# ClashLuke/LocAtE

Hardware: AMD Instinct MI355X
Metric: images/sec (G+D step) 64x64 bs=64 (higher is better)
Workload: dtype f32 (contractions fp32-faithful on the matrix cores: 2 x scaled fp16 operand pieces / 3 MFMAs per slice where the operand's largest magnitude comes with it, else 3 x bf16 pieces / 6 MFMAs; fp32 accumulate); 1 GPU; LocAtE G+D step, 64x64 RGB, batch 64 per GPU (the fp32 variant - the reference's own precision - of BASELINE.json configs[1]: 64x64 RGB bs 64), self/feature attention at 16x16 and 64x64, random-init weights; global_batch=64, image_size=64, parallelism=dp1, launch=hipGraph replay, G-step generator pass on a second stream

## Files before the change

include/locate_hip.h:

```cpp
#ifndef LOCATE_HIP_H
#define LOCATE_HIP_H
#include <stddef.h>
#include <stdint.h>
#ifdef __cplusplus
extern "C" {
#endif

const char* locate_last_error(void);
int locate_abi_version(void);
int locate_device_info(char* arch_name, int name_len, int* cu_count, int* wave_size);

int locate_roottanh_fwd(const float* x, float* y, int64_t n, void* absmax , void* stream);
int locate_absmax_words(void);
int locate_roottanh_bwd(const float* x, const float* gy, float* gx, int64_t n, int accumulate, void* absmax, void* stream);
int locate_absmax(const float* x, int64_t n, void* absmax, void* stream);
int locate_act_cat_rows_fwd(const float* latent, const float* pre, float* out, int rows, int z, int w, void* stream);
int locate_act_rows_bwd(const float* pre, const float* g, int64_t g_row_stride, const float* g_add, float* gpre, int rows, int w,
                        void* stream);
int locate_add3(const float* a, int64_t a_bs, const float* b, int64_t b_bs, const float* c, int64_t c_bs, float* out, int batch,
                int64_t per, void* stream);
int locate_tanh_fwd(const float* x, float* y, int64_t n, void* stream);
int locate_tanh_bwd(const float* y, const float* gy, float* gx, int64_t n, void* stream);

size_t locate_norm_stats_workspace_bytes(void);
// ... 47 lines not shown
                         const float* wv, float* gw, float* du, float* dsigma_out, int h, int wd, void* stream);
size_t locate_sn_group_workspace_bytes(void);
int locate_sn_weight_bwd_grouped(const float* gy, int64_t gy_bs, const float* y, int64_t y_bs, const float* bias, int groups,
                                 int Bg, int M, int plane, const float* sigma_tab, int sigma_stride, const float* u,
                                 const float* v, const float* wv, int64_t wv_stride, float* gw, float* du,
                                 float* dsigma_total_out, int h, int wd, void* workspace, void* stream);
int locate_sn_dv_batched(const void* table, int n_layers, int max_h, int max_wd, void* stream);

size_t locate_conv_panel_bytes(const int* geom, int adjoint);
int locate_conv_pack_panel(const int* geom, int adjoint, const float* w, float* panel, void* stream);
size_t locate_conv_pack_job_bytes(void);
int locate_conv_pack_job(const int* geom, int adjoint, const float* w, float* panel, int block_start, void* job_out,
                         int* blocks_out, int direct, const void* weight_absmax);
int locate_conv_pack_panels(const void* jobs, int n_jobs, int total_blocks, int any_f16, int passes, void* stream);
int locate_conv_pack_job_is_direct(const void* job);
int locate_conv_pack_job_is_window(const void* job);
int locate_conv_win_ok(const int* geom, int adjoint_fmt, int64_t x_bs, const void* x);
size_t locate_conv_win_workspace_bytes(const int* geom, int adjoint_fmt);
size_t locate_conv_fwd_workspace_bytes(const int* geom);
size_t locate_conv_counter_bytes(void);
int locate_conv_fwd(const int* geom, const float* x, int64_t x_bs, const float* panel, const float* scale,
                    int scale_group_batch, int scale_stride, const float* bias, float* y, int64_t y_bs, void* workspace,
                    void* counters, int precision, const void* x_absmax, const void* act_epilogue, void* stream);
size_t locate_conv_dgrad_workspace_bytes(const int* geom);
int locate_conv_dgrad(const int* geom, const float* gy, int64_t gy_bs, const float* panel, const float* scale,
                      int scale_group_batch, int scale_stride, const float* bias, float* gx, int64_t gx_bs, void* workspace,
                      void* counters, int precision, const void* gy_absmax, const void* act_epilogue, void* stream);
size_t locate_conv_wgrad_workspace_bytes(const int* geom);
int locate_conv_wgrad_partials(const int* geom);
int locate_conv_wgrad(const int* geom, const float* x, int64_t x_bs, const float* gy, int64_t gy_bs, float* gw,
                      const float* w_ref, const float* inv_scale, int scale_group_batch, int scale_stride,
                      double* inner_partial, void* workspace, int precision, const void* x_absmax, const void* gy_absmax,
                      void* deferred_reduce, void* stream);
int locate_conv_wgrad_group_partials(const int* geom, int groups);
size_t locate_conv_wgrad_group_workspace_bytes(const int* geom, int groups);
size_t locate_slab_reduce_record_bytes(void);
int locate_slab_reduce_max(void);
int locate_slab_reduce_record_blocks(const void* record);
int locate_slab_reduce_batch(const void* records, int n, void* stream);

size_t locate_wgrad_batch_record_bytes(void);
int locate_wgrad_batch_max(void);
int locate_wgrad_batch_record(const int* geom, const float* x, int64_t x_bs, const float* gy, int64_t gy_bs, float* gw,
                              const float* w_ref, const float* inv_scale, int scale_group_batch, int scale_stride,
                              double* inner_partial, void* record);
int locate_wgrad_batch(const void* records, int n, void* stream);

int locate_dwconv_fwd(const int* geom, const float* x, int64_t x_bs, const float* w, const float* scale, int scale_group_batch,
                      int scale_stride, float* y, int64_t y_bs, void* stream);
int locate_dwconv_dgrad(const int* geom, const float* gy, int64_t gy_bs, const float* w, const float* scale,
                        int scale_group_batch, int scale_stride, float* gx, int64_t gx_bs, void* stream);
size_t locate_dwconv_wgrad_workspace_bytes(const int* geom);
int locate_dwconv_wgrad_partials(const int* geom);
int locate_dwconv_wgrad(const int* geom, const float* big, int64_t big_bs, const float* small, int64_t small_bs, float* gw,
                        const float* w_ref, const float* inv_scale, int scale_group_batch, int scale_stride,
                        double* inner_partial, void* workspace, void* stream);
int locate_groupdot_fwd(const float* x, int64_t x_bs, const float* w, const float* scale, int scale_group_batch,
                        int scale_stride, float* y, int B, int G, int L, void* stream);
int locate_groupdot_dgrad(const float* gy, const float* w, const float* scale, int scale_group_batch, int scale_stride,
                          float* gx, int64_t gx_bs, int B, int G, int L, void* stream);
int locate_groupdot_wgrad_partials(int G, int L);
int locate_groupdot_wgrad(const float* x, int64_t x_bs, const float* gy, float* gw, const float* w_ref, const float* inv_scale,
                          int scale_group_batch, int scale_stride, double* inner_partial, int B, int G, int L, void* stream);

size_t locate_fin_record_bytes(void);
int locate_fin_sn_dot_partials(int Bg, int M, int plane);
// ... 49 lines not shown
```

locate_amd/_lib.py:

```python
import ctypes
import os

import torch

_HERE = os.path.dirname(os.path.abspath(__file__))
LIB_PATH = os.path.join(_HERE, "csrc", "liblocate_hip_dbg.so" if os.environ.get("LOCATE_HIP_DEBUG_LIBRARY") == "1"
                        else "liblocate_hip.so")

c_p = ctypes.c_void_p
c_i = ctypes.c_int
c_i64 = ctypes.c_int64
c_f = ctypes.c_float
c_d = ctypes.c_double
c_sz = ctypes.c_size_t
c_ip = ctypes.POINTER(ctypes.c_int)

PROTOTYPES = {
    "locate_last_error": (ctypes.c_char_p, []),
    "locate_abi_version": (c_i, []),
    "locate_device_info": (c_i, [ctypes.c_char_p, c_i, c_ip, c_ip]),
    "locate_roottanh_fwd": (c_i, [c_p, c_p, c_i64, c_p, c_p]),
    "locate_roottanh_bwd": (c_i, [c_p, c_p, c_p, c_i64, c_i, c_p, c_p]),
    "locate_act_cat_rows_fwd": (c_i, [c_p, c_p, c_p, c_i, c_i, c_i, c_p]),
    "locate_act_rows_bwd": (c_i, [c_p, c_p, c_i64, c_p, c_p, c_i, c_i, c_p]),
# ... 28 lines not shown
    "locate_pool2_upsample2x_fwd": (c_i, [c_p, c_p, c_i64, c_i, c_i, c_p]),
    "locate_pool2_upsample2x_bwd": (c_i, [c_p, c_p, c_i64, c_i, c_i, c_i, c_p]),
    "locate_avgpool2_fwd": (c_i, [c_p, c_p, c_i64, c_i, c_i, c_p]),
    "locate_avgpool2_bwd": (c_i, [c_p, c_p, c_i64, c_i, c_i, c_i, c_p]),
    "locate_feature_pool_fwd": (c_i, [c_p, c_p, c_i64, c_i, c_p]),
    "locate_feature_pool_bwd": (c_i, [c_p, c_p, c_i64, c_i, c_i, c_p]),
    "locate_copy_channels": (c_i, [c_p, c_p, c_i, c_i, c_i, c_i64, c_i64, c_i, c_p]),
    "locate_sn_workspace_bytes": (c_sz, [c_i, c_i]),
    "locate_sn_power_iter": (c_i, [c_p, c_p, c_p, c_p, c_p, c_i, c_i, c_p, c_p]),
    "locate_sn_table_record_bytes": (c_sz, []),
    "locate_sn_power_iter_batched": (c_i, [c_p, c_i, c_i, c_i, c_p]),
    "locate_sn_weight_bwd": (c_i, [c_p, c_i, c_p, c_p, c_p, c_p, c_p, c_p, c_p, c_i, c_i, c_p]),
    "locate_sn_group_workspace_bytes": (c_sz, []),
    "locate_sn_weight_bwd_grouped": (c_i, [c_p, c_i64, c_p, c_i64, c_p, c_i, c_i, c_i, c_i, c_p, c_i, c_p, c_p, c_p, c_i64, c_p,
                                           c_p, c_p, c_i, c_i, c_p, c_p]),
    "locate_sn_dv_batched": (c_i, [c_p, c_i, c_i, c_i, c_p]),
    "locate_conv_panel_bytes": (c_sz, [c_ip, c_i]),
    "locate_conv_pack_panel": (c_i, [c_ip, c_i, c_p, c_p, c_p]),
    "locate_conv_pack_job_bytes": (c_sz, []),
    "locate_conv_pack_job": (c_i, [c_ip, c_i, c_p, c_p, c_i, c_p, c_ip, c_i, c_p]),
    "locate_conv_pack_panels": (c_i, [c_p, c_i, c_i, c_i, c_i, c_p]),
    "locate_conv_pack_job_is_direct": (c_i, [c_p]),
    "locate_conv_pack_job_is_window": (c_i, [c_p]),
    "locate_conv_win_ok": (c_i, [c_ip, c_i, c_i64, c_p]),
    "locate_conv_win_workspace_bytes": (c_sz, [c_ip, c_i]),
    "locate_conv_fwd_workspace_bytes": (c_sz, [c_ip]),
    "locate_conv_counter_bytes": (c_sz, []),
    "locate_conv_fwd": (c_i, [c_ip, c_p, c_i64, c_p, c_p, c_i, c_i, c_p, c_p, c_i64, c_p, c_p, c_i, c_p, c_p, c_p]),
    "locate_conv_dgrad_workspace_bytes": (c_sz, [c_ip]),
    "locate_conv_dgrad": (c_i, [c_ip, c_p, c_i64, c_p, c_p, c_i, c_i, c_p, c_p, c_i64, c_p, c_p, c_i, c_p, c_p, c_p]),
    "locate_conv_wgrad_workspace_bytes": (c_sz, [c_ip]),
    "locate_conv_wgrad_partials": (c_i, [c_ip]),
    "locate_conv_wgrad": (c_i, [c_ip, c_p, c_i64, c_p, c_i64, c_p, c_p, c_p, c_i, c_i, c_p, c_p, c_i, c_p, c_p, c_p, c_p]),
    "locate_conv_wgrad_group_partials": (c_i, [c_ip, c_i]),
    "locate_conv_wgrad_group_workspace_bytes": (c_sz, [c_ip, c_i]),
    "locate_slab_reduce_record_bytes": (c_sz, []),
    "locate_slab_reduce_max": (c_i, []),
    "locate_slab_reduce_record_blocks": (c_i, [c_p]),
    "locate_slab_reduce_batch": (c_i, [c_p, c_i, c_p]),
    "locate_dwconv_fwd": (c_i, [c_ip, c_p, c_i64, c_p, c_p, c_i, c_i, c_p, c_i64, c_p]),
    "locate_dwconv_dgrad": (c_i, [c_ip, c_p, c_i64, c_p, c_p, c_i, c_i, c_p, c_i64, c_p]),
    "locate_dwconv_wgrad_workspace_bytes": (c_sz, [c_ip]),
    "locate_dwconv_wgrad_partials": (c_i, [c_ip]),
    "locate_dwconv_wgrad": (c_i, [c_ip, c_p, c_i64, c_p, c_i64, c_p, c_p, c_p, c_i, c_i, c_p, c_p, c_p]),
    "locate_groupdot_fwd": (c_i, [c_p, c_i64, c_p, c_p, c_i, c_i, c_p, c_i, c_i, c_i, c_p]),
    "locate_groupdot_dgrad": (c_i, [c_p, c_p, c_p, c_i, c_i, c_p, c_i64, c_i, c_i, c_i, c_p]),
    "locate_groupdot_wgrad_partials": (c_i, [c_i, c_i]),
    "locate_groupdot_wgrad": (c_i, [c_p, c_i64, c_p, c_p, c_p, c_p, c_i, c_i, c_p, c_i, c_i, c_i, c_p]),
    "locate_fin_record_bytes": (c_sz, []),
    "locate_fin_sn_dot_partials": (c_i, [c_i, c_i, c_i]),
    "locate_fin_sn_dots": (c_i, [c_p, c_i, c_p]),
    "locate_fin_sn_rank1": (c_i, [c_p, c_i, c_p]),
    "locate_fin_sums": (c_i, [c_p, c_i, c_p]),
    "locate_fin_channel_slices": (c_i, [c_i, c_i, c_i]),
    "locate_fin_channel_sums": (c_i, [c_p, c_i, c_p]),
    "locate_gate_bwd_partials": (c_i, [c_i64, c_i]),
    "locate_multi_copy_record_bytes": (c_sz, []),
    "locate_multi_copy_chunk_elems": (c_i, []),
    "locate_multi_copy": (c_i, [c_p, c_p, c_i, c_i, c_f, c_p]),
    "locate_nadam_tensor_record_bytes": (c_sz, []),
    "locate_nadam_chunk_elems": (c_i, []),
    "locate_nadam_step": (c_i, [c_p, c_p, c_p, c_i, c_i, c_d, c_d, c_d, c_d, c_d, c_d, c_p]),
    "locate_average_record_bytes": (c_sz, []),
    "locate_average_chunk_elems": (c_i, []),
    "locate_average_update": (c_i, [c_p, c_p, c_i, c_i, c_p]),
    "locate_d_loss": (c_i, [c_p, c_p, c_p, c_i, c_f, c_p, c_p, c_p, c_p, c_p]),
# ... 64 lines not shown
```

locate_amd/build.py:

```python
import os
import shutil
import subprocess
import sys

CSRC = os.path.join(os.path.dirname(os.path.abspath(__file__)), "csrc")
LIB = os.path.join(CSRC, "liblocate_hip.so")
LIB_DBG = os.path.join(CSRC, "liblocate_hip_dbg.so")
DBG_SOURCES = ["conv.hip", "convwgrad.hip", "convwin.hip"]
SOURCES = ["runtime.hip", "elementwise.hip", "norm.hip", "softmax.hip", "resample.hip", "spectral.hip", "conv.hip", "convpack.hip", "convwgrad.hip", "convwin.hip", "convfp8.hip",
           "grouped.hip", "nadam.hip", "loss.hip", "finalise.hip", "parallel.hip", "input.hip", "grid.hip", "swd.hip", "average.hip"]
ARCH = "gfx950"


def _hipcc():
    for cand in (os.environ.get("HIPCC"), shutil.which("hipcc"), "/opt/rocm/bin/hipcc"):
        if cand and os.path.exists(cand):
            return cand
    raise RuntimeError("hipcc not found: the MI355X kernels cannot be built")


def _sources():
    return [s for s in SOURCES if os.path.exists(os.path.join(CSRC, s))]


def _headers():
    return [os.path.join(CSRC, h) for h in sorted(os.listdir(CSRC)) if h.endswith(".h")]


def needs_build():
    if not (os.path.exists(LIB) and os.path.exists(LIB_DBG)):
        return True
    t = min(os.path.getmtime(LIB), os.path.getmtime(LIB_DBG))
    deps = [os.path.join(CSRC, s) for s in _sources()] + _headers()
    return any(os.path.getmtime(d) > t for d in deps)


def build(force=False, verbose=True):
    if not force and not needs_build():
        return LIB
    hipcc = _hipcc()
    objs = []
    flags = ["--offload-arch=" + ARCH, "-O3", "-fPIC", "-std=c++17", "-fvisibility=hidden", "-Wall", "-Wno-unused-function",
# ... 39 lines not shown
```

locate_amd/csrc/convwgrad.hip:

```cpp
#include "igemm.h"

#define WG_BK 32

struct WgParams {
    const float* x;
    const float* gy;
    float* slab;
    long long x_bs, gy_bs;
    unsigned x_bytes;
    int B, C, H, W, M, OH, OW, KH, KW, stride, pad_h, pad_w;
    int R;
    int N;
    int chunk;
    int zper, Ng;
    unsigned q_mul, ow_mul;
    int q_s1, q_s2, ow_s1, ow_s2;
    int gscale_bg, gscale_stride;
    float* direct_out;
    const float* w_ref;
    const float* inv_scale;
    double* partial;
    const unsigned* x_absmax;
    const unsigned* g_absmax;
};


template <int WGM, int WGN, int TM, int TN>
__device__ __forceinline__ void wgrad_epilogue(const WgParams& p, f32x16 (&acc)[TM][TN], int r0, int m0, int wm, int wn, int lane,
                                               int wid, int tid) {
    const int lrow = lane >> 5, lcol = lane & 31;
    __shared__ double red[4];
    const bool direct = p.direct_out != nullptr;
    float* dst = direct ? p.direct_out : p.slab + (long long)blockIdx.z * p.M * p.R;
// ... 1101 lines not shown
    int scale_bg, scale_stride, N, M, C, grid_x, block0;
    OnePix op;
};
#define SKW_MAX 24
struct SkwBatch {
    SkwRec r[SKW_MAX];
};

__global__ void __launch_bounds__(256) skinny_wgrad_batch_kernel(const SkwBatch b, int n) {
    int k = 0;
    for (int i = 1; i < n; ++i)
        if ((int)blockIdx.x >= b.r[i].block0) k = i;
    const SkwRec& r = b.r[k];
    const int local = (int)blockIdx.x - r.block0;
    const int by = local / r.grid_x, bx = local - by * r.grid_x;
    if (r.M >= SKW_WIDE_M)
        skinny_wgrad_wide(r.x, r.x_bs, r.gy, r.gy_bs, r.gw, r.w_ref, r.inv_scale, r.scale_bg, r.scale_stride, r.partial, r.N, r.M, r.C,
                          r.op, bx, by, r.grid_x);
    else
        skinny_wgrad_body<SKW_MT>(r.x, r.x_bs, r.gy, r.gy_bs, r.gw, r.w_ref, r.inv_scale, r.scale_bg, r.scale_stride, r.partial, r.N, r.M,
                                  r.C, r.op, bx, by, r.grid_x);
}

static bool skinny_wgrad_ok(const ConvGeom& g) {
    return !path_disabled("skinny") && g.KH == 1 && g.KW == 1 && g.stride == 1 && g.pad_h == 0 && g.pad_w == 0 && g.H == 1 &&
           g.W == 1 && g.OH == 1 && g.OW == 1;
}
static dim3 skinny_wgrad_grid(const ConvGeom& g) { return dim3((g.C + 63) / 64, (g.M + skw_mt(g.M) - 1) / skw_mt(g.M)); }
static bool onepix_wgrad_ok(const ConvGeom& g) {
    return !path_disabled("skinny") && !skinny_wgrad_ok(g) && g.OH == 1 && g.OW == 1 && (long long)g.C * g.H * g.W < (1 << 24);
}
static dim3 onepix_wgrad_grid(const ConvGeom& g) { return dim3((g.C * g.H * g.W + 63) / 64, (g.M + skw_mt(g.M) - 1) / skw_mt(g.M)); }

enum WgradKind { WG_MAP1X1, WG_ONEPIX, WG_POINTWISE, WG_TILED };
struct WgradRoute {
    WgradKind kind;
    dim3 grid;
    int bm;
    PwPlan pw;
    int nsplit, chunk, zper;
    int64_t n;
    int partials;
    size_t ws_bytes;
    bool dots;
};

static WgradRoute wgrad_route(const ConvGeom& g, int groups) {
    WgradRoute r;
    const bool stacked = groups >= 2 && groups <= 4 && g.B % groups == 0;
    if (!stacked) groups = 0;
    r.bm = 0; r.nsplit = 1; r.chunk = 0; r.zper = 1; r.partials = 0; r.ws_bytes = 0; r.dots = false;
    r.n = (int64_t)g.M * g.C * g.KH * g.KW;
    const bool map1x1 = skinny_wgrad_ok(g);
    if (map1x1 || onepix_wgrad_ok(g)) {
        r.kind = map1x1 ? WG_MAP1X1 : WG_ONEPIX;
        r.grid = map1x1 ? skinny_wgrad_grid(g) : onepix_wgrad_grid(g);
        r.partials = (int)(r.grid.x * r.grid.y);
        return r;
    }
    r.pw = pw_plan(g, groups);
    if (r.pw.ok) {
        r.kind = WG_POINTWISE;
        if (stacked && r.pw.zper == 0) return r;
        r.nsplit = r.pw.nslab; r.chunk = r.pw.chunk; r.zper = r.pw.zper;
        r.grid = dim3(r.pw.nslab, r.pw.tiles_m * r.pw.tiles_c);
        r.dots = stacked;
    } else {
        r.kind = WG_TILED;
        int tiles;
        wgrad_plan(g, groups, &r.bm, &r.nsplit, &r.chunk, &r.zper, &tiles);
        r.grid = dim3((g.C * g.KH * g.KW + 127) / 128, (g.M + r.bm - 1) / r.bm, r.nsplit);
        r.dots = stacked && (long long)g.B * g.OH * g.OW < (1ll << 31);
        if (r.nsplit == 1) { r.partials = tiles; return r; }
    }
    r.partials = wgrad_reduce_grid(r.n, r.nsplit);
    r.ws_bytes = (size_t)r.nsplit * r.n * sizeof(float);
    return r;
}

LOCATE_API size_t locate_conv_wgrad_workspace_bytes(const int* geom) { return wgrad_route(make_geom(geom), 0).ws_bytes; }

LOCATE_API int locate_conv_wgrad_partials(const int* geom) { return wgrad_route(make_geom(geom), 0).partials; }

LOCATE_API size_t locate_wgrad_batch_record_bytes(void) { return sizeof(SkwRec); }
LOCATE_API int locate_wgrad_batch_max(void) { return SKW_MAX; }
LOCATE_API int locate_wgrad_batch_record(const int* geom, const float* x, int64_t x_bs, const float* gy, int64_t gy_bs, float* gw,
                                         const float* w_ref, const float* inv_scale, int scale_group_batch, int scale_stride,
                                         double* inner_partial, void* record) {
    const ConvGeom g = make_geom(geom);
    if (geom_check(g, "locate_wgrad_batch_record") || !record || !x || !gy || !gw) return 0;
    if (inner_partial && !w_ref) return 0;
    if (scale_group_batch < 0 || (scale_group_batch > 0 && (!inv_scale || g.B % scale_group_batch != 0 || g.B / scale_group_batch > 4 ||
                                                            w_ref || inner_partial))) return 0;
    const WgradRoute route = wgrad_route(g, 0);
    if (route.kind != WG_MAP1X1 && route.kind != WG_ONEPIX) return 0;
    const bool skinny = route.kind == WG_MAP1X1;
    const dim3 grid = route.grid;
    SkwRec r;
    r.x = x; r.gy = gy; r.gw = gw; r.w_ref = w_ref; r.inv_scale = inv_scale; r.partial = inner_partial;
    r.x_bs = x_bs; r.gy_bs = gy_bs;
    r.scale_bg = scale_group_batch; r.scale_stride = scale_stride; r.N = g.B; r.M = g.M; r.C = skinny ? g.C : g.C * g.H * g.W;
    r.grid_x = (int)grid.x; r.block0 = 0;
    r.op = skinny ? OnePix{0, 0, 0, 0, 0, 0, 0} : OnePix{g.H * g.W, g.W, g.KH, g.KW, g.pad_h, g.pad_w, g.C};
    memcpy(record, &r, sizeof(r));
    return (int)(grid.x * grid.y);
}
LOCATE_API int locate_wgrad_batch(const void* records, int n, void* stream) {
    LOCATE_REQUIRE(records && n > 0 && n <= SKW_MAX, "locate_wgrad_batch: 1 .. locate_wgrad_batch_max() records");
    SkwBatch b;
    memcpy(b.r, records, (size_t)n * sizeof(SkwRec));
    long long blocks = 0;
    for (int i = 0; i < n; ++i) {
        const SkwRec& r = b.r[i];
        LOCATE_REQUIRE(r.x && r.gy && r.gw && r.grid_x > 0 && r.M > 0 && r.C > 0 && r.N > 0, "locate_wgrad_batch: bad record");
        b.r[i].block0 = (int)blocks;
        blocks += (long long)r.grid_x * ((r.M + skw_mt(r.M) - 1) / skw_mt(r.M));
    }
    LOCATE_REQUIRE(blocks < (1ll << 31), "locate_wgrad_batch: too many blocks");
    skinny_wgrad_batch_kernel<<<(unsigned)blocks, 256, 0, as_stream(stream)>>>(b, n);
    LOCATE_LAUNCH_CHECK("locate_wgrad_batch");
    return LOCATE_OK;
}

LOCATE_API int locate_conv_wgrad_group_partials(const int* geom, int groups) {
    const ConvGeom g = make_geom(geom);
    if (geom_check(g, "locate_conv_wgrad_group_partials")) return 0;
    const WgradRoute r = wgrad_route(g, groups);
    return r.dots ? r.partials : 0;
}
LOCATE_API size_t locate_conv_wgrad_group_workspace_bytes(const int* geom, int groups) {
    const ConvGeom g = make_geom(geom);
    if (geom_check(g, "locate_conv_wgrad_group_workspace_bytes")) return 0;
    const WgradRoute r = wgrad_route(g, groups);
    return r.dots ? r.ws_bytes : 0;
}

template <int NP>
static void launch_wgrad_bx6(const WgParams& p, dim3 grid, int bm, hipStream_t st) {
    with_tile<true>(bm, [&](auto t) { using T = decltype(t); conv_wgrad_bx6_kernel<T::wgm, T::wgn, T::tm, T::tn, NP><<<grid, 256, 0, st>>>(p); });
}

LOCATE_API int locate_conv_wgrad(const int* geom, const float* x, int64_t x_bs, const float* gy, int64_t gy_bs, float* gw,
                                 const float* w_ref, const float* inv_scale, int scale_group_batch, int scale_stride,
                                 double* inner_partial, void* workspace, int precision, const void* x_absmax, const void* gy_absmax,
                                 void* deferred_reduce, void* stream) {
    const ConvGeom g = make_geom(geom);
    if (int e = geom_check(g, "locate_conv_wgrad")) return e;
    LOCATE_REQUIRE(precision >= 0 && precision <= 3, "locate_conv_wgrad: precision must be 0 (fp32-faithful, bf16 pieces), 1 (bf16 operands), 2 (fp32-faithful, fp16 pieces) or 3 (fp8 operands)");
    LOCATE_REQUIRE(precision < 2 || (x_absmax && gy_absmax), "locate_conv_wgrad: precisions 2 and 3 need the absmax words of x and gy");
    LOCATE_REQUIRE(x && gy && gw, "locate_conv_wgrad: null pointer");
    LOCATE_REQUIRE(!inner_partial || w_ref, "locate_conv_wgrad: inner_partial needs w_ref");
    const int gd = (scale_group_batch > 0 && w_ref && inner_partial && g.B % scale_group_batch == 0) ? g.B / scale_group_batch : 0;
    const WgradRoute r = wgrad_route(g, gd);
    LOCATE_REQUIRE(scale_group_batch >= 0 && (scale_group_batch == 0 || (inv_scale && g.B % scale_group_batch == 0 &&
                   g.B / scale_group_batch <= 4 && ((!w_ref && !inner_partial) || r.dots))),
                   "locate_conv_wgrad: bad group scaling arguments (per-call partials: see locate_conv_wgrad_group_partials)");
    hipStream_t st = as_stream(stream);
    if (deferred_reduce) memset(deferred_reduce, 0, sizeof(SlabRec));
    auto reduce = [&](const float* slab, const float* scale, const char* who) -> int {
        const int64_t n = r.n;
        const int nsplit = r.nsplit, zper = r.zper, rg = r.partials;
        const int zp = wgrad_reduce_zp(nsplit, n);
        if (deferred_reduce) {
            SlabRec rec;
            rec.slab = slab; rec.out = gw; rec.w_ref = w_ref; rec.inv_scale = scale; rec.partial = inner_partial;
            rec.n = n; rec.nsplit = nsplit; rec.zp = zp; rec.grid = rg; rec.block0 = 0; rec.groups = gd; rec.zper = zper;
            memcpy(deferred_reduce, &rec, sizeof(rec));
            return LOCATE_OK;
        }
        if (zp == 16) slab_reduce_kernel<16><<<rg, 256, 0, st>>>(slab, gw, n, nsplit, w_ref, scale, inner_partial, gd, zper);
        else if (zp == 4) slab_reduce_kernel<4><<<rg, 256, 0, st>>>(slab, gw, n, nsplit, w_ref, scale, inner_partial, gd, zper);
        else slab_reduce_kernel<1><<<rg, 256, 0, st>>>(slab, gw, n, nsplit, w_ref, scale, inner_partial, gd, zper);
        LOCATE_LAUNCH_CHECK(who);
        return LOCATE_OK;
    };
    if (r.kind == WG_MAP1X1) {
        skinny_wgrad_kernel<<<r.grid, 256, 0, st>>>(x, x_bs, gy, gy_bs, gw, w_ref, inv_scale, scale_group_batch, scale_stride,
                                                   inner_partial, g.B, g.M, g.C, OnePix{0, 0, 0, 0, 0, 0, 0});
        LOCATE_LAUNCH_CHECK("locate_conv_wgrad(1x1 map)");
        return LOCATE_OK;
    }
    if (r.kind == WG_ONEPIX) {
        const OnePix op = {g.H * g.W, g.W, g.KH, g.KW, g.pad_h, g.pad_w, g.C};
        skinny_wgrad_kernel<<<r.grid, 256, 0, st>>>(x, x_bs, gy, gy_bs, gw, w_ref, inv_scale, scale_group_batch, scale_stride,
                                                   inner_partial, g.B, g.M, g.C * g.H * g.W, op);
        LOCATE_LAUNCH_CHECK("locate_conv_wgrad(one output pixel)");
        return LOCATE_OK;
    }
    const dim3 grid = r.grid;
    if (r.kind == WG_POINTWISE) {
        const PwPlan& pq = r.pw;
        LOCATE_REQUIRE((x_bs & 3) == 0 && (gy_bs & 3) == 0 &&
                       ((reinterpret_cast<uintptr_t>(x) | reinterpret_cast<uintptr_t>(gy)) & 15) == 0,
                       "locate_conv_wgrad: narrow 1x1 layers need 16-byte aligned x / gy and batch strides that are multiples of 4");
        LOCATE_REQUIRE(workspace, "locate_conv_wgrad: the split reduction needs a workspace");
        PwParams q;
        q.x = x; q.gy = gy; q.slab = static_cast<float*>(workspace); q.x_bs = x_bs; q.gy_bs = gy_bs;
        q.B = g.B; q.C = g.C; q.M = g.M; q.P = g.H * g.W; q.N = g.B * g.H * g.W; q.steps = pq.steps; q.chunk = pq.chunk;
        q.tiles_c = pq.tiles_c;
        const bool grouped = scale_group_batch > 0;
        q.inv_scale = grouped ? inv_scale : nullptr; q.gscale_bg = scale_group_batch; q.gscale_stride = scale_stride;
        const int key = (pq.tm - 1) * 2 + (pq.tn - 1);
        q.x_absmax = static_cast<const unsigned*>(x_absmax);
        q.g_absmax = static_cast<const unsigned*>(gy_absmax);
        if (precision == 2 && x_absmax && gy_absmax && !grouped) {
            if (key == 0) pw_wgrad_kernel<1, 1, 2><<<grid, 256, 0, st>>>(q);
            else if (key == 1) pw_wgrad_kernel<1, 2, 2><<<grid, 256, 0, st>>>(q);
            else if (key == 2) pw_wgrad_kernel<2, 1, 2><<<grid, 256, 0, st>>>(q);
            else pw_wgrad_kernel<2, 2, 2><<<grid, 256, 0, st>>>(q);
        } else if (precision == 1) {
            if (key == 0) pw_wgrad_kernel<1, 1, 1><<<grid, 256, 0, st>>>(q);
            else if (key == 1) pw_wgrad_kernel<1, 2, 1><<<grid, 256, 0, st>>>(q);
            else if (key == 2) pw_wgrad_kernel<2, 1, 1><<<grid, 256, 0, st>>>(q);
            else pw_wgrad_kernel<2, 2, 1><<<grid, 256, 0, st>>>(q);
        } else {
            if (key == 0) pw_wgrad_kernel<1, 1, 3><<<grid, 256, 0, st>>>(q);
            else if (key == 1) pw_wgrad_kernel<1, 2, 3><<<grid, 256, 0, st>>>(q);
            else if (key == 2) pw_wgrad_kernel<2, 1, 3><<<grid, 256, 0, st>>>(q);
            else pw_wgrad_kernel<2, 2, 3><<<grid, 256, 0, st>>>(q);
        }
        LOCATE_LAUNCH_CHECK("locate_conv_wgrad(pointwise)");
        return reduce(q.slab, grouped ? nullptr : inv_scale, "locate_conv_wgrad(pointwise reduce)");
    }
    const int bm = r.bm, nsplit = r.nsplit, chunk = r.chunk, zper = r.zper;
    LOCATE_REQUIRE(nsplit == 1 || workspace, "locate_conv_wgrad: split reduction needs a workspace");
    WgParams p;
    p.x = x; p.gy = gy; p.slab = static_cast<float*>(workspace); p.x_bs = x_bs; p.gy_bs = gy_bs;
    p.B = g.B; p.C = g.C; p.H = g.H; p.W = g.W; p.M = g.M; p.OH = g.OH; p.OW = g.OW; p.KH = g.KH; p.KW = g.KW;
    p.stride = g.stride; p.pad_h = g.pad_h; p.pad_w = g.pad_w;
    p.R = g.C * g.KH * g.KW; p.N = g.B * g.OH * g.OW; p.chunk = chunk;
    p.zper = zper; p.Ng = gd > 1 ? p.N / gd : p.N;
    fastdiv_make((unsigned)(g.OH * g.OW), &p.q_mul, &p.q_s1, &p.q_s2);
    fastdiv_make((unsigned)g.OW, &p.ow_mul, &p.ow_s1, &p.ow_s2);
    const bool direct = nsplit == 1;
    const bool grouped = scale_group_batch > 0;
    p.gscale_bg = scale_group_batch; p.gscale_stride = scale_stride;
    p.x_absmax = static_cast<const unsigned*>(x_absmax);
    p.g_absmax = static_cast<const unsigned*>(gy_absmax);
    p.direct_out = direct ? gw : nullptr;
    p.w_ref = direct ? w_ref : nullptr;
    p.inv_scale = (direct || grouped) ? inv_scale : nullptr;
    p.partial = direct ? inner_partial : nullptr;
    const long long x_extent = 4ll * ((long long)(g.B - 1) * x_bs + (long long)g.C * g.H * g.W);
    p.x_bytes = (unsigned)x_extent;
    const bool pairs_ok = ((g.OH * g.OW) & 1) == 0 && (g.OW & 1) == 0 && (gy_bs & 1) == 0 && (chunk & 1) == 0 &&
                          (reinterpret_cast<uintptr_t>(gy) & 7) == 0 && x_extent > 0 && x_extent < (1ll << 31) - (1 << 20);
    LOCATE_REQUIRE(bm != 192 || pairs_ok, "locate_conv_wgrad: layers with M %% 192 == 0 on even maps take the paired-load kernels - gy must be 8-byte aligned with an even batch stride");
    const bool bx6 = pairs_ok && (precision == 1 || precision == 3 || !path_disabled("wbx6"));
    if (bx6 && precision == 3) launch_wgrad_bx6<4>(p, grid, bm, st);
    else if (bx6 && precision == 1) launch_wgrad_bx6<1>(p, grid, bm, st);
    else if (bx6 && precision == 2) launch_wgrad_bx6<2>(p, grid, bm, st);
    else if (bx6) launch_wgrad_bx6<3>(p, grid, bm, st);
    else
        with_tile<false>(bm, [&](auto t) { using T = decltype(t); conv_wgrad_kernel<T::wgm, T::wgn, T::tm, T::tn><<<grid, 256, 0, st>>>(p); });
    LOCATE_LAUNCH_CHECK("locate_conv_wgrad(gemm)");
    if (!direct) return reduce(p.slab, grouped ? nullptr : inv_scale, "locate_conv_wgrad(reduce)");
    return LOCATE_OK;
}
// ... 26 lines not shown
```

Measured before the change: 7158 images/sec.

## Add row-band conv weight-gradient kernel reusing LDS input rows across output rows

Adds a new wgrad kernel for 3x3 stride-1 convolutions at 64-wide maps with few output channels. Each block walks a band of output rows and keeps a ring of KH+S input rows in LDS as split fp16 hi/lo pieces, so each input row is loaded once and reused across kernel offsets. The next row's loads are double-buffered against the MFMAs. Partial results go to a split slab reduced by the existing reduce kernel, at the cost of larger workspace, more split partials and up to 80KB of dynamic LDS per block.

```diff
diff --git a/include/locate_hip.h b/include/locate_hip.h
--- a/include/locate_hip.h
+++ b/include/locate_hip.h
@@ -103,6 +103,7 @@
                       const float* w_ref, const float* inv_scale, int scale_group_batch, int scale_stride,
                       double* inner_partial, void* workspace, int precision, const void* x_absmax, const void* gy_absmax,
                       void* deferred_reduce, void* stream);
+long long locate_conv_wgrad_band_launches(void);
 int locate_conv_wgrad_group_partials(const int* geom, int groups);
 size_t locate_conv_wgrad_group_workspace_bytes(const int* geom, int groups);
 size_t locate_slab_reduce_record_bytes(void);
diff --git a/locate_amd/_lib.py b/locate_amd/_lib.py
--- a/locate_amd/_lib.py
+++ b/locate_amd/_lib.py
@@ -84,6 +84,7 @@
     "locate_conv_wgrad_workspace_bytes": (c_sz, [c_ip]),
     "locate_conv_wgrad_partials": (c_i, [c_ip]),
     "locate_conv_wgrad": (c_i, [c_ip, c_p, c_i64, c_p, c_i64, c_p, c_p, c_p, c_i, c_i, c_p, c_p, c_i, c_p, c_p, c_p, c_p]),
+    "locate_conv_wgrad_band_launches": (ctypes.c_longlong, []),
     "locate_conv_wgrad_group_partials": (c_i, [c_ip, c_i]),
     "locate_conv_wgrad_group_workspace_bytes": (c_sz, [c_ip, c_i]),
     "locate_slab_reduce_record_bytes": (c_sz, []),
diff --git a/locate_amd/build.py b/locate_amd/build.py
--- a/locate_amd/build.py
+++ b/locate_amd/build.py
@@ -6,8 +6,8 @@
 CSRC = os.path.join(os.path.dirname(os.path.abspath(__file__)), "csrc")
 LIB = os.path.join(CSRC, "liblocate_hip.so")
 LIB_DBG = os.path.join(CSRC, "liblocate_hip_dbg.so")
-DBG_SOURCES = ["conv.hip", "convwgrad.hip", "convwin.hip"]
-SOURCES = ["runtime.hip", "elementwise.hip", "norm.hip", "softmax.hip", "resample.hip", "spectral.hip", "conv.hip", "convpack.hip", "convwgrad.hip", "convwin.hip", "convfp8.hip",
+DBG_SOURCES = ["conv.hip", "convwgrad.hip", "convwin.hip", "convband.hip"]
+SOURCES = ["runtime.hip", "elementwise.hip", "norm.hip", "softmax.hip", "resample.hip", "spectral.hip", "conv.hip", "convpack.hip", "convwgrad.hip", "convband.hip", "convwin.hip", "convfp8.hip",
            "grouped.hip", "nadam.hip", "loss.hip", "finalise.hip", "parallel.hip", "input.hip", "grid.hip", "swd.hip", "average.hip"]
 ARCH = "gfx950"
 
diff --git a/locate_amd/csrc/convband.h b/locate_amd/csrc/convband.h
--- /dev/null
+++ b/locate_amd/csrc/convband.h
@@ -0,0 +1,21 @@
+#pragma once
+#include "igemm.h"
+
+#define BAND_LDS_BYTES (80 * 1024)
+
+struct BandPlan {
+    int ok;
+    int cb;
+    int tm;
+    int tiles_r, tiles_m;
+    int zper, rpb;
+    int nsplit;
+    int lds_bytes;
+};
+
+BandPlan band_plan(const ConvGeom& g, int groups);
+bool band_default(const ConvGeom& g);
+bool band_operands_ok(const float* gy, long long gy_bs);
+int band_launch(const ConvGeom& g, const BandPlan& plan, int groups, const float* x, long long x_bs, const float* gy, long long gy_bs,
+                float* slab, const float* inv_scale, int scale_group_batch, int scale_stride, const unsigned* x_absmax,
+                const unsigned* g_absmax, hipStream_t st);
diff --git a/locate_amd/csrc/convband.hip b/locate_amd/csrc/convband.hip
--- /dev/null
+++ b/locate_amd/csrc/convband.hip
@@ -0,0 +1,364 @@
+#include "convband.h"
+
+struct BandParams {
+    const float* x;
+    const float* gy;
+    float* slab;
+    long long x_bs, gy_bs;
+    int B, C, H, W, M, OH, OW, KH, KW, stride, pad_h, pad_w;
+    int R, cb, nch, zper, rpb, rows_per_call;
+    int gscale_bg, gscale_stride;
+    const float* inv_scale;
+    const unsigned* x_absmax;
+    const unsigned* g_absmax;
+};
+
+#define BAND_GPT 3
+#define BAND_XPT 2
+
+__device__ __forceinline__ float band_group_scale(int b, int bg, float gs0, float gs1, float gs2, float gs3) {
+    float gsc = gs0;
+    gsc = b >= bg ? gs1 : gsc;
+    gsc = b >= 2 * bg ? gs2 : gsc;
+    gsc = b >= 3 * bg ? gs3 : gsc;
+    return gsc;
+}
+
+__device__ __forceinline__ void band_load_x8(const float* __restrict__ rowp, int ix0, int s, int W, bool row_ok, float (&v)[8]) {
+#pragma unroll
+    for (int j = 0; j < 8; ++j) {
+        const int ix = ix0 + j * s;
+        const int ixc = min(max(ix, 0), W - 1);
+        const unsigned keep = (row_ok && (unsigned)ix < (unsigned)W) ? 0xffffffffu : 0u;
+        v[j] = __uint_as_float(__float_as_uint(rowp[ixc]) & keep);
+    }
+}
+
+__device__ __forceinline__ void band_load_g8(const float* __restrict__ src, float mul, float (&v)[8]) {
+    const float4 t0 = *reinterpret_cast<const float4*>(src), t1 = *reinterpret_cast<const float4*>(src + 4);
+    v[0] = t0.x * mul; v[1] = t0.y * mul; v[2] = t0.z * mul; v[3] = t0.w * mul;
+    v[4] = t1.x * mul; v[5] = t1.y * mul; v[6] = t1.z * mul; v[7] = t1.w * mul;
+}
+
+__device__ __forceinline__ void band_write_chunk(uint4* smem, const float (&v)[8], float sc, int dst, int plane, int trash) {
+    uint4 h, l;
+    split2_f16x8(v, sc, h, l);
+    smem[dst >= 0 ? dst : trash] = h;
+    smem[dst >= 0 ? dst + plane : trash] = l;
+}
+
+__device__ __forceinline__ void band_write_row3(uint4* smem, const float (&v)[8], float sc, unsigned keep, bool left, bool right, int dst,
+                                                int XP, int plane, int trash) {
+    uint4 h, l;
+    split2_f16x8(v, sc, h, l);
+    h.x &= keep; h.y &= keep; h.z &= keep; h.w &= keep;
+    l.x &= keep; l.y &= keep; l.z &= keep; l.w &= keep;
+    unsigned hp = __shfl_up(h.w, 1), lp = __shfl_up(l.w, 1), hn = __shfl_down(h.x, 1), ln = __shfl_down(l.x, 1);
+    hp = left ? 0u : hp; lp = left ? 0u : lp;
+    hn = right ? 0u : hn; ln = right ? 0u : ln;
+    const unsigned h01 = __builtin_amdgcn_alignbyte(h.y, h.x, 2), h12 = __builtin_amdgcn_alignbyte(h.z, h.y, 2), h23 = __builtin_amdgcn_alignbyte(h.w, h.z, 2);
+    const unsigned l01 = __builtin_amdgcn_alignbyte(l.y, l.x, 2), l12 = __builtin_amdgcn_alignbyte(l.z, l.y, 2), l23 = __builtin_amdgcn_alignbyte(l.w, l.z, 2);
+    const int d0 = dst >= 0 ? dst : trash, d1 = dst >= 0 ? dst + XP : trash, d2 = dst >= 0 ? dst + 2 * XP : trash;
+    const int pl = dst >= 0 ? plane : 0;
+    smem[d0] = make_uint4(__builtin_amdgcn_alignbyte(h.x, hp, 2), h01, h12, h23);
+    smem[d1] = h;
+    smem[d2] = make_uint4(h01, h12, h23, __builtin_amdgcn_alignbyte(hn, h.w, 2));
+    smem[d0 + pl] = make_uint4(__builtin_amdgcn_alignbyte(l.x, lp, 2), l01, l12, l23);
+    smem[d1 + pl] = l;
+    smem[d2 + pl] = make_uint4(l01, l12, l23, __builtin_amdgcn_alignbyte(ln, l.w, 2));
+}
+
+template <int TM, int KS>
+__device__ __forceinline__ void band_mfma_row(const uint4* smem, f32x16 (&acc)[TM], int bs, int x_plane, int ga, int g_plane, int lrow, int nks) {
+    constexpr int BM = TM * 32;
+    auto slice = [&](int ks) {
+        const int owc = 2 * ks + lrow;
+        const f16x8 bh = *reinterpret_cast<const f16x8*>(&smem[bs + owc]);
+        const f16x8 bl = *reinterpret_cast<const f16x8*>(&smem[x_plane + bs + owc]);
+#pragma unroll
+        for (int i = 0; i < TM; ++i) {
+            const f16x8 ah = *reinterpret_cast<const f16x8*>(&smem[ga + owc * (BM + 1) + i * 32]);
+            const f16x8 al = *reinterpret_cast<const f16x8*>(&smem[ga + g_plane + owc * (BM + 1) + i * 32]);
+            acc[i] = __builtin_amdgcn_mfma_f32_32x32x16_f16(al, bh, acc[i], 0, 0, 0);
+            acc[i] = __builtin_amdgcn_mfma_f32_32x32x16_f16(ah, bl, acc[i], 0, 0, 0);
+            acc[i] = __builtin_amdgcn_mfma_f32_32x32x16_f16(ah, bh, acc[i], 0, 0, 0);
+        }
+    };
+    if constexpr (KS > 0) {
+#pragma unroll
+        for (int ks = 0; ks < KS; ++ks) slice(ks);
+    } else {
+        for (int ks = 0; ks < nks; ++ks) slice(ks);
+    }
+}
+
+template <int TM, bool FAST, int KS>
+__global__ void __launch_bounds__(256, 2) conv_wgrad_band_kernel(const BandParams p) {
+    constexpr int BM = TM * 32;
+    extern __shared__ uint4 smem[];
+    const int tid = threadIdx.x, lane = tid & 63, wid = tid >> 6;
+    const int lrow = lane >> 5, lcol = lane & 31;
+    const int T = p.KH * p.KW, S = p.stride;
+    const int NCH = p.nch, NCHE = (NCH + 1) & ~1, XP = NCH + 1, NR = p.KH + S;
+    const int c0 = blockIdx.x * p.cb, m0 = blockIdx.y * BM;
+    const int cbe = min(p.cb, p.C - c0);
+    const int Q = p.OH * p.OW;
+    const int slot_pitch = p.KW * XP;
+    const int x_plane = p.cb * NR * slot_pitch;
+    const int g_plane = NCHE * (BM + 1);
+    const int g_base = 2 * x_plane;
+    const int trash = g_base + 4 * g_plane;
+    for (int i = tid; i <= trash; i += 256) smem[i] = make_uint4(0u, 0u, 0u, 0u);
+
+    float gs0 = 1.0f, gs1 = 1.0f, gs2 = 1.0f, gs3 = 1.0f;
+    if (p.gscale_bg > 0) {
+        const int ng = p.B / p.gscale_bg;
+        gs0 = p.inv_scale[0];
+        gs1 = ng > 1 ? p.inv_scale[p.gscale_stride] : 1.0f;
+        gs2 = ng > 2 ? p.inv_scale[2 * p.gscale_stride] : 1.0f;
+        gs3 = ng > 3 ? p.inv_scale[3 * p.gscale_stride] : 1.0f;
+    }
+    const float gmax = __uint_as_float(absmax_read(p.g_absmax)) * fmaxf(fmaxf(gs0, gs1), fmaxf(gs2, gs3));
+    const int kg_ = f16_scale_exp(__float_as_uint(gmax) + (p.gscale_bg > 0 ? 0x00800000u : 0u));
+    const int kx_ = f16_scale_exp(absmax_read(p.x_absmax));
+    const float g_scale = pow2f(kg_), x_scale = pow2f(kx_);
+    float g_unscale, x_unscale;
+    unscale_pair(kg_, kx_, g_unscale, x_unscale);
+
+    int g_src[BAND_GPT], g_dst[BAND_GPT];
+#pragma unroll
+    for (int i = 0; i < BAND_GPT; ++i) {
+        const int id = tid + 256 * i;
+        const int m = id / NCH, owc = id - m * NCH;
+        const bool ok = id < BM * NCH && m0 + m < p.M;
+        g_src[i] = ok ? (m0 + m) * Q + owc * 8 : 0;
+        g_dst[i] = ok ? g_base + owc * (BM + 1) + m : -1;
+    }
+    int x_src[BAND_XPT], x_ix0[BAND_XPT], x_rr[BAND_XPT], x_dst[BAND_XPT];
+#pragma unroll
+    for (int i = 0; i < BAND_XPT; ++i) {
+        const int id = tid + 256 * i;
+        int t = id / NCH;
+        const int owc = id - t * NCH;
+        const int kx = t % p.KW; t /= p.KW;
+        const int rr = t % S, cl = t / S;
+        const bool ok = cl < cbe;
+        x_src[i] = ok ? (c0 + cl) * p.H * p.W : 0;
+        x_ix0[i] = owc * 8 * S + kx - p.pad_w;
+        x_rr[i] = rr;
+        x_dst[i] = ok ? cl * NR * slot_pitch + kx * XP + owc : -1;
+    }
+    const int col = wid * 32 + lcol;
+    const bool col_ok = col < cbe * T;
+    const int colc = col_ok ? col : 0;
+    const int b_cl = colc / T, b_t = colc - b_cl * T;
+    const int b_ky = b_t / p.KW, b_kx = b_t - b_ky * p.KW;
+    const int b_off = b_cl * NR * slot_pitch + b_kx * XP;
+
+    f32x16 acc[TM];
+#pragma unroll
+    for (int i = 0; i < TM; ++i)
+#pragma unroll
+        for (int e = 0; e < 16; ++e) acc[i][e] = 0.0f;
+
+    const int call = (int)blockIdx.z / p.zper, band = (int)blockIdx.z - call * p.zper;
+    const int row_begin = call * p.rows_per_call + band * p.rpb;
+    const int row_end = min(row_begin + p.rpb, (call + 1) * p.rows_per_call);
+
+    const int bg = p.gscale_bg > 0 ? p.gscale_bg : (1 << 29);
+
+    const int fcl = tid / NCH, fq = tid - fcl * NCH;
+    const bool f_ok = fcl < cbe;
+    const bool f_wave = __builtin_amdgcn_readfirstlane(tid >> 6) * 64 < p.cb * NCH;
+    const int f_src = f_ok ? (c0 + fcl) * p.H * p.W + 8 * fq : 0;
+    const int f_dst = f_ok ? fcl * NR * slot_pitch + fq : -1;
+    const bool f_left = fq == 0, f_right = fq == NCH - 1;
+    const bool xpt2 = p.cb * S * p.KW * NCH > 256;
+
+    constexpr int GP = KS > 0 ? (TM * KS + 3) / 4 : BAND_GPT;
+    const bool gpt2 = KS > 0 ? GP > 1 : BM * NCH > 256, gpt3 = KS > 0 ? GP > 2 : BM * NCH > 512;
+    float gv0[8], gv1[8], gv2[8], xv0[8], xv1[8];
+#define BAND_LOADS(OHN)                                                                                                            \
+    {                                                                                                                              \
+        const float* gb_ = gyb + (OHN) * p.OW;                                                                                     \
+        const int un_ = (OHN) * S + p.KH - S;                                                                                      \
+        band_load_g8(gb_ + g_src[0], gsc, gv0);                                                                                    \
+        if (gpt2) band_load_g8(gb_ + g_src[1], gsc, gv1);                                                                          \
+        if (gpt3) band_load_g8(gb_ + g_src[2], gsc, gv2);                                                                          \
+        if constexpr (FAST) {                                                                                                      \
+            if (KS > 0 || f_wave) band_load_g8(xb + f_src + min(max(un_ - p.pad_h, 0), p.H - 1) * p.W, 1.0f, xv0);                 \
+        } else {                                                                                                                   \
+            const int iy0_ = un_ + x_rr[0] - p.pad_h;                                                                              \
+            band_load_x8(xb + x_src[0] + min(max(iy0_, 0), p.H - 1) * p.W, x_ix0[0], S, p.W, (unsigned)iy0_ < (unsigned)p.H, xv0); \
+            if (xpt2) {                                                                                                            \
+                const int iy1_ = un_ + x_rr[1] - p.pad_h;                                                                          \
+                band_load_x8(xb + x_src[1] + min(max(iy1_, 0), p.H - 1) * p.W, x_ix0[1], S, p.W, (unsigned)iy1_ < (unsigned)p.H, xv1); \
+            }                                                                                                                      \
+        }                                                                                                                          \
+    }
+
+    bool need_full = true, have_next = false;
+    int buf = 0;
+    for (int row = row_begin; row < row_end; ++row) {
+        const int b = row / p.OH, oh = row - b * p.OH;
+        const float* xb = p.x + (long long)b * p.x_bs;
+        const float* gyb = p.gy + (long long)b * p.gy_bs;
+        const float gsc = band_group_scale(b, bg, gs0, gs1, gs2, gs3);
+        if (need_full) {
+            __syncthreads();
+            if constexpr (FAST) {
+                if (f_wave) {
+                    for (int ky = 0; ky < p.KH; ++ky) {
+                        const int u = oh + ky, iy = u - p.pad_h, iyc = min(max(iy, 0), p.H - 1);
+                        float v[8];
+                        band_load_g8(xb + f_src + iyc * p.W, 1.0f, v);
+                        band_write_row3(smem, v, x_scale, (unsigned)iy < (unsigned)p.H ? 0xffffffffu : 0u, f_left, f_right,
+                                        f_dst >= 0 ? f_dst + (u % NR) * slot_pitch : -1, XP, x_plane, trash);
+                    }
+                }
+            } else {
+                const int items = cbe * p.KH * p.KW * NCH;
+                for (int id = tid; id < items; id += 256) {
+                    int t = id / NCH;
+                    const int owc = id - t * NCH;
+                    const int kx = t % p.KW; t /= p.KW;
+                    const int ky = t % p.KH, cl = t / p.KH;
+                    const int u = oh * S + ky, iy = u - p.pad_h;
+                    const int iyc = min(max(iy, 0), p.H - 1);
+                    float v[8];
+                    band_load_x8(xb + (c0 + cl) * p.H * p.W + iyc * p.W, owc * 8 * S + kx - p.pad_w, S, p.W, (unsigned)iy < (unsigned)p.H, v);
+                    band_write_chunk(smem, v, x_scale, (cl * NR + u % NR) * slot_pitch + kx * XP + owc, x_plane, trash);
+                }
+            }
+            const float* gb = gyb + oh * p.OW;
+            const int gofs = buf * 2 * g_plane;
+#pragma unroll
+            for (int i = 0; i < BAND_GPT; ++i) {
+                float v[8];
+                band_load_g8(gb + g_src[i], gsc, v);
+                band_write_chunk(smem, v, g_scale, g_dst[i] >= 0 ? g_dst[i] + gofs : -1, g_plane, trash);
+            }
+            __syncthreads();
+        }
+        const bool same_img = row + 1 < row_end && oh + 1 < p.OH;
+        if (same_img && !have_next) BAND_LOADS(oh + 1)
+
+        const int bs = b_off + ((oh * S + b_ky) % NR) * slot_pitch;
+        const int ga = g_base + buf * 2 * g_plane + lcol;
+        if (same_img) {
+            const int u_new = (oh + 1) * S + p.KH - S;
+            const int gofs = (buf ^ 1) * 2 * g_plane;
+            band_mfma_row<TM, KS>(smem, acc, bs, x_plane, ga, g_plane, lrow, NCHE / 2);
+            band_write_chunk(smem, gv0, g_scale, g_dst[0] >= 0 ? g_dst[0] + gofs : -1, g_plane, trash);
+            if (gpt2) band_write_chunk(smem, gv1, g_scale, g_dst[1] >= 0 ? g_dst[1] + gofs : -1, g_plane, trash);
+            if (gpt3) band_write_chunk(smem, gv2, g_scale, g_dst[2] >= 0 ? g_dst[2] + gofs : -1, g_plane, trash);
+            if constexpr (FAST) {
+                if (KS > 0 || f_wave)
+                    band_write_row3(smem, xv0, x_scale, (unsigned)(u_new - p.pad_h) < (unsigned)p.H ? 0xffffffffu : 0u, f_left, f_right,
+                                    f_dst >= 0 ? f_dst + (u_new % NR) * slot_pitch : -1, XP, x_plane, trash);
+            } else {
+                band_write_chunk(smem, xv0, x_scale, x_dst[0] >= 0 ? x_dst[0] + ((u_new + x_rr[0]) % NR) * slot_pitch : -1, x_plane, trash);
+                if (xpt2)
+                    band_write_chunk(smem, xv1, x_scale, x_dst[1] >= 0 ? x_dst[1] + ((u_new + x_rr[1]) % NR) * slot_pitch : -1, x_plane, trash);
+            }
+            buf ^= 1;
+        } else {
+            band_mfma_row<TM, KS>(smem, acc, bs, x_plane, ga, g_plane, lrow, NCHE / 2);
+        }
+        have_next = same_img && row + 2 < row_end && oh + 2 < p.OH;
+        if (have_next) BAND_LOADS(oh + 2)
+        need_full = !same_img;
+        __syncthreads();
+    }
+#undef BAND_LOADS
+
+    float* dst = p.slab + (long long)blockIdx.z * p.M * p.R;
+    const int r = c0 * T + col;
+#pragma unroll
+    for (int i = 0; i < TM; ++i)
+#pragma unroll
+        for (int e = 0; e < 16; ++e) {
+            const int m = m0 + i * 32 + (e & 3) + 8 * (e >> 2) + 4 * lrow;
+            if (col_ok && m < p.M) dst[(long long)m * p.R + r] = (acc[i][e] * g_unscale) * x_unscale;
+        }
+}
+
+BandPlan band_plan(const ConvGeom& g, int groups) {
+    BandPlan p;
+    memset(&p, 0, sizeof(p));
+    const int T = g.KH * g.KW, S = g.stride;
+    const int calls = groups > 1 ? groups : 1;
+    if (S < 1 || S > 2 || g.OW % 8 != 0 || g.OW < 16 || T > 128 || g.B % calls != 0) return p;
+    if ((int64_t)g.B * g.OH >= (1 << 30)) return p;
+    const int NCH = g.OW / 8, NCHE = (NCH + 1) & ~1, NR = g.KH + S;
+    int cb = 128 / T;
+    if (cb > g.C) cb = g.C;
+    const int tiles_r = (g.C + cb - 1) / cb;
+    cb = (g.C + tiles_r - 1) / tiles_r;
+    int bm = 96, best_pad = 1 << 30;
+    const int cands[3] = {96, 64, 32};
+    for (int i = 0; i < 3; ++i) {
+        const int pad = round_up(g.M, cands[i]);
+        if (pad < best_pad) { best_pad = pad; bm = cands[i]; }
+    }
+    if (bm * NCH > 256 * BAND_GPT || cb * S * g.KW * NCH > 256 * BAND_XPT) return p;
+    const int64_t chunks = 2ll * cb * NR * g.KW * (NCH + 1) + 4ll * NCHE * (bm + 1) + 1;
+    if (chunks * 16 > BAND_LDS_BYTES) return p;
+    const int tiles_m = (g.M + bm - 1) / bm;
+    const int rows = (g.B / calls) * g.OH;
+    const int target = knob_int("LOCATE_BAND_BLOCKS", 512);
+    int zper = target / (tiles_r * tiles_m * calls);
+    if (zper > rows / 4) zper = rows / 4;
+    if (zper < 1) zper = 1;
+    const int rpb = (rows + zper - 1) / zper;
+    zper = (rows + rpb - 1) / rpb;
+    p.ok = 1; p.cb = cb; p.tm = bm / 32; p.tiles_r = tiles_r; p.tiles_m = tiles_m; p.zper = zper; p.rpb = rpb;
+    p.nsplit = calls * zper;
+    p.lds_bytes = (int)(chunks * 16);
+    return p;
+}
+
+bool band_default(const ConvGeom& g) {
+    return g.KH == 3 && g.KW == 3 && g.stride == 1 && g.pad_w == 1 && g.OW == 64 && g.M <= 64;
+}
+
+bool band_operands_ok(const float* gy, long long gy_bs) { return (reinterpret_cast<uintptr_t>(gy) & 15) == 0 && (gy_bs & 3) == 0; }
+
+template <int TM, bool FAST, int KS = 0>
+static void band_launch_tm(const BandParams& q, dim3 grid, int lds, hipStream_t st) {
+    auto k = conv_wgrad_band_kernel<TM, FAST, KS>;
+    static bool enabled = false;
+    if (!enabled) { (void)hipFuncSetAttribute(reinterpret_cast<const void*>(k), hipFuncAttributeMaxDynamicSharedMemorySize, BAND_LDS_BYTES); enabled = true; }
+    k<<<grid, 256, lds, st>>>(q);
+}
+
+int band_launch(const ConvGeom& g, const BandPlan& plan, int groups, const float* x, long long x_bs, const float* gy, long long gy_bs,
+                float* slab, const float* inv_scale, int scale_group_batch, int scale_stride, const unsigned* x_absmax,
+                const unsigned* g_absmax, hipStream_t st) {
+    LOCATE_REQUIRE(plan.ok && x && gy && slab && x_absmax && g_absmax, "locate_conv_wgrad(band): no plan or null pointer");
+    LOCATE_REQUIRE(band_operands_ok(gy, gy_bs), "locate_conv_wgrad(band): gy must be 16-byte aligned with a batch stride that is a multiple of 4");
+    const int calls = groups > 1 ? groups : 1;
+    BandParams q;
+    q.x = x; q.gy = gy; q.slab = slab; q.x_bs = x_bs; q.gy_bs = gy_bs;
+    q.B = g.B; q.C = g.C; q.H = g.H; q.W = g.W; q.M = g.M; q.OH = g.OH; q.OW = g.OW; q.KH = g.KH; q.KW = g.KW;
+    q.stride = g.stride; q.pad_h = g.pad_h; q.pad_w = g.pad_w;
+    q.R = g.C * g.KH * g.KW; q.cb = plan.cb; q.nch = g.OW / 8; q.zper = plan.zper; q.rpb = plan.rpb;
+    q.rows_per_call = (g.B / calls) * g.OH;
+    q.gscale_bg = scale_group_batch; q.gscale_stride = scale_stride; q.inv_scale = inv_scale;
+    q.x_absmax = x_absmax; q.g_absmax = g_absmax;
+    const dim3 grid(plan.tiles_r, plan.tiles_m, plan.nsplit);
+    const bool fast = g.stride == 1 && g.KW == 3 && g.pad_w == 1 && 64 % q.nch == 0 && (reinterpret_cast<uintptr_t>(x) & 15) == 0 &&
+                      (x_bs & 3) == 0 && knob_int("LOCATE_BAND_FAST", 1);
+    if (fast) {
+        if (plan.tm == 3) band_launch_tm<3, true>(q, grid, plan.lds_bytes, st);
+        else if (plan.tm == 2 && q.nch == 8) band_launch_tm<2, true, 4>(q, grid, plan.lds_bytes, st);
+        else if (plan.tm == 2) band_launch_tm<2, true>(q, grid, plan.lds_bytes, st);
+        else band_launch_tm<1, true>(q, grid, plan.lds_bytes, st);
+    } else {
+        if (plan.tm == 3) band_launch_tm<3, false>(q, grid, plan.lds_bytes, st);
+        else if (plan.tm == 2) band_launch_tm<2, false>(q, grid, plan.lds_bytes, st);
+        else band_launch_tm<1, false>(q, grid, plan.lds_bytes, st);
+    }
+    LOCATE_LAUNCH_CHECK("locate_conv_wgrad(band)");
+    return LOCATE_OK;
+}
diff --git a/locate_amd/csrc/convwgrad.hip b/locate_amd/csrc/convwgrad.hip
--- a/locate_amd/csrc/convwgrad.hip
+++ b/locate_amd/csrc/convwgrad.hip
@@ -1,4 +1,5 @@
 #include "igemm.h"
+#include "convband.h"
 
 #define WG_BK 32
 
@@ -1166,7 +1167,7 @@
 }
 static dim3 onepix_wgrad_grid(const ConvGeom& g) { return dim3((g.C * g.H * g.W + 63) / 64, (g.M + skw_mt(g.M) - 1) / skw_mt(g.M)); }
 
-enum WgradKind { WG_MAP1X1, WG_ONEPIX, WG_POINTWISE, WG_TILED };
+enum WgradKind { WG_MAP1X1, WG_ONEPIX, WG_POINTWISE, WG_TILED, WG_BAND };
 struct WgradRoute {
     WgradKind kind;
     dim3 grid;
@@ -1177,12 +1178,14 @@
     int partials;
     size_t ws_bytes;
     bool dots;
+    BandPlan band;
 };
 
 static WgradRoute wgrad_route(const ConvGeom& g, int groups) {
     WgradRoute r;
     const bool stacked = groups >= 2 && groups <= 4 && g.B % groups == 0;
     if (!stacked) groups = 0;
+    r.band.ok = 0;
     r.bm = 0; r.nsplit = 1; r.chunk = 0; r.zper = 1; r.partials = 0; r.ws_bytes = 0; r.dots = false;
     r.n = (int64_t)g.M * g.C * g.KH * g.KW;
     const bool map1x1 = skinny_wgrad_ok(g);
@@ -1206,9 +1209,11 @@
         r.grid = dim3((g.C * g.KH * g.KW + 127) / 128, (g.M + r.bm - 1) / r.bm, r.nsplit);
         r.dots = stacked && (long long)g.B * g.OH * g.OW < (1ll << 31);
         if (r.nsplit == 1) { r.partials = tiles; return r; }
+        if (!path_disabled("band")) r.band = band_plan(g, groups);
+        if (r.band.ok) r.kind = WG_BAND;
     }
     r.partials = wgrad_reduce_grid(r.n, r.nsplit);
-    r.ws_bytes = (size_t)r.nsplit * r.n * sizeof(float);
+    r.ws_bytes = (size_t)(r.band.ok && r.band.nsplit > r.nsplit ? r.band.nsplit : r.nsplit) * r.n * sizeof(float);
     return r;
 }
 
@@ -1269,6 +1274,9 @@
     return r.dots ? r.ws_bytes : 0;
 }
 
+static long long band_launches = 0;
+LOCATE_API long long locate_conv_wgrad_band_launches(void) { return __atomic_load_n(&band_launches, __ATOMIC_RELAXED); }
+
 template <int NP>
 static void launch_wgrad_bx6(const WgParams& p, dim3 grid, int bm, hipStream_t st) {
     with_tile<true>(bm, [&](auto t) { using T = decltype(t); conv_wgrad_bx6_kernel<T::wgm, T::wgn, T::tm, T::tn, NP><<<grid, 256, 0, st>>>(p); });
@@ -1280,6 +1288,8 @@
                                  void* deferred_reduce, void* stream) {
     const ConvGeom g = make_geom(geom);
     if (int e = geom_check(g, "locate_conv_wgrad")) return e;
+    const bool force_band = (precision & 32) != 0, no_band = (precision & 64) != 0;
+    precision &= ~(32 | 64);
     LOCATE_REQUIRE(precision >= 0 && precision <= 3, "locate_conv_wgrad: precision must be 0 (fp32-faithful, bf16 pieces), 1 (bf16 operands), 2 (fp32-faithful, fp16 pieces) or 3 (fp8 operands)");
     LOCATE_REQUIRE(precision < 2 || (x_absmax && gy_absmax), "locate_conv_wgrad: precisions 2 and 3 need the absmax words of x and gy");
     LOCATE_REQUIRE(x && gy && gw, "locate_conv_wgrad: null pointer");
@@ -1291,9 +1301,10 @@
                    "locate_conv_wgrad: bad group scaling arguments (per-call partials: see locate_conv_wgrad_group_partials)");
     hipStream_t st = as_stream(stream);
     if (deferred_reduce) memset(deferred_reduce, 0, sizeof(SlabRec));
+    int rd_nsplit = r.nsplit, rd_zper = r.zper;
     auto reduce = [&](const float* slab, const float* scale, const char* who) -> int {
         const int64_t n = r.n;
-        const int nsplit = r.nsplit, zper = r.zper, rg = r.partials;
+        const int nsplit = rd_nsplit, zper = rd_zper, rg = r.partials;
         const int zp = wgrad_reduce_zp(nsplit, n);
         if (deferred_reduce) {
             SlabRec rec;
@@ -1358,6 +1369,15 @@
     }
     const int bm = r.bm, nsplit = r.nsplit, chunk = r.chunk, zper = r.zper;
     LOCATE_REQUIRE(nsplit == 1 || workspace, "locate_conv_wgrad: split reduction needs a workspace");
+    if (r.kind == WG_BAND && precision == 2 && x_absmax && gy_absmax && band_operands_ok(gy, gy_bs) && !no_band && (force_band || band_default(g))) {
+        const bool grouped_ = scale_group_batch > 0;
+        if (int e = band_launch(g, r.band, gd, x, x_bs, gy, gy_bs, static_cast<float*>(workspace), grouped_ ? inv_scale : nullptr,
+                                scale_group_batch, scale_stride, static_cast<const unsigned*>(x_absmax),
+                                static_cast<const unsigned*>(gy_absmax), st)) return e;
+        __atomic_fetch_add(&band_launches, 1ll, __ATOMIC_RELAXED);
+        rd_nsplit = r.band.nsplit; rd_zper = r.band.zper;
+        return reduce(static_cast<const float*>(workspace), grouped_ ? nullptr : inv_scale, "locate_conv_wgrad(band reduce)");
+    }
     WgParams p;
     p.x = x; p.gy = gy; p.slab = static_cast<float*>(workspace); p.x_bs = x_bs; p.gy_bs = gy_bs;
     p.B = g.B; p.C = g.C; p.H = g.H; p.W = g.W; p.M = g.M; p.OH = g.OH; p.OW = g.OW; p.KH = g.KH; p.KW = g.KW;
```

Result: no change. 7188 images/sec, median of 6 (+0.4%).
